# NVlabs/FoundationPose

Hardware: AMD Instinct MI355X
Metric: pose-hypotheses/sec (raster+refine+score), 252 hyp x 160x160 @ 640x480 RGB-D (higher is better)
Workload: dtype f16

## Files before the change

### foundationpose_amd/_lib.py

```python
import ctypes as C
import os

import torch

_HERE = os.path.dirname(os.path.abspath(__file__))
LIB_PATH = os.environ.get("FP_AMD_LIB") or os.path.join(_HERE, "csrc", "libfp_amd.so")
ABI_VERSION = 223
_lib = None

vp, ci, cf, cd, sz = C.c_void_p, C.c_int, C.c_float, C.c_double, C.c_size_t

SIGNATURES = {
    "fp_last_error": (C.c_char_p, []),
    "fp_version": (ci, []),
    "fp_mesh_create": (ci, [vp, vp, vp, vp, vp, vp, vp, ci, ci, ci, ci, C.POINTER(vp)]),
    "fp_mesh_destroy": (None, [vp]),
    "fp_mesh_set_create": (ci, [vp, ci, C.POINTER(vp)]),
    "fp_mesh_set_destroy": (None, [vp]),
    "fp_mesh_set_workspace_bytes": (sz, [vp, ci, ci, ci]),
    "fp_depth_erode": (ci, [vp, vp, ci, ci, ci, cf, cf, cf, vp]),
    "fp_depth_bilateral": (ci, [vp, vp, ci, ci, ci, cf, cf, cf, vp]),
    "fp_depth_to_xyz": (ci, [vp, vp, cf, ci, vp, ci, ci, vp]),
    "fp_crop_windows": (ci, [vp, vp, cd, cd, ci, ci, ci, vp, vp, vp]),
    "fp_crop_windows_multi": (ci, [vp, vp, vp, vp, ci, cd, ci, ci, ci, vp, vp, vp]),
    "fp_depth_erode_frames": (ci, [vp, vp, ci, ci, ci, ci, cf, cf, cf, vp]),
    "fp_depth_bilateral_frames": (ci, [vp, vp, ci, ci, ci, ci, cf, cf, cf, vp]),
    "fp_depth_to_xyz_frames": (ci, [vp, vp, cf, ci, vp, ci, ci, ci, vp]),
    "fp_mask_depth_stats": (ci, [vp, vp, vp, ci, ci, ci, ci, cf, vp, vp]),
    "fp_crop_windows_views": (ci, [vp, vp, vp, ci, vp, vp, ci, cd, ci, ci, ci, vp, vp, vp]),
    "fp_render_crops_views": (ci, [vp, vp, vp, vp, vp, ci, vp, vp, ci, ci, ci, ci, ci, cf, cf, cf, ci, vp, vp, vp, vp, vp, vp, vp, vp, sz, vp]),
    "fp_warp_crops_views": (ci, [vp, vp, vp, vp, vp, vp, ci, vp, vp, vp, ci, ci, ci, ci, ci, ci, ci, ci, vp, vp]),
    "fp_pose_update_views": (ci, [vp, vp, vp, ci, ci, vp, cf, vp, vp, ci, ci, vp, vp, vp, ci, vp, vp, ci, vp, cf, vp]),
    "fp_depth_agreement": (ci, [vp, vp, vp, vp, ci, ci, ci, ci, ci, ci, cf, vp, vp]),
    "fp_pose_errors_workspace_bytes": (sz, [ci, ci, ci]),
    "fp_pose_errors": (ci, [vp, ci, vp, ci, vp, vp, vp, ci, ci, ci, vp, vp, sz, vp]),
    "fp_vsd_counts": (ci, [vp, vp, vp, ci, ci, ci, ci, vp, vp, ci, ci, ci, ci, cf, vp, ci, vp, vp]),
    "fp_mspd": (ci, [vp, ci, vp, ci, vp, vp, vp, ci, ci, vp, vp, vp]),
    "fp_tsdf_integrate": (ci, [vp, vp, vp, vp, vp, ci, ci, ci, ci, ci, ci, vp, cf, cf, cf, vp, vp, vp, vp, vp]),
    "fp_tsdf_count_triangles": (ci, [vp, vp, ci, ci, ci, cf, vp, vp]),
    "fp_tsdf_emit_triangles": (ci, [vp, vp, vp, vp, ci, ci, ci, vp, cf, cf, vp, C.c_longlong, vp, vp, vp, vp, vp]),
    "fp_texture_bake": (ci, [vp, ci, vp, ci, vp, vp, vp, vp, vp, vp, ci, ci, ci, ci, ci, cf, cf, cf, vp, vp, vp]),
    "fp_workspace_bytes": (sz, [ci, ci, ci, ci, ci]),
    "fp_render_crops": (ci, [vp, vp, vp, vp, ci, ci, ci, ci, ci, cf, cf, cf, cf, ci, vp, vp, vp, vp, vp, vp, vp, vp, sz, vp]),
    "fp_render_crops_multi": (ci, [vp, vp, vp, vp, vp, vp, ci, ci, ci, ci, ci, cf, cf, cf, ci, vp, vp, vp, vp, vp, vp, vp, vp, sz, vp]),
    "fp_warp_crops": (ci, [vp, vp, vp, vp, vp, vp, cf, ci, ci, ci, ci, ci, ci, ci, vp, vp]),
    "fp_warp_crops_multi": (ci, [vp, vp, vp, vp, vp, vp, vp, vp, ci, ci, ci, ci, ci, ci, ci, ci, vp, vp]),
    "fp_pose_update": (ci, [vp, vp, vp, ci, ci, vp, cf, cf, ci, vp, vp, vp, ci, vp, vp, cf, vp]),
    "fp_pose_update_multi": (ci, [vp, vp, vp, ci, ci, vp, cf, vp, vp, ci, ci, vp, vp, vp, ci, vp, vp, cf, vp]),
    "fp_conv7x7s2_bn_relu_fwd": (ci, [vp, vp, vp, vp, vp, vp, ci, ci, ci, ci, vp]),
    "fp_igemm_f16_fwd": (ci, [vp, vp, vp, vp, vp, ci, ci, ci, ci, vp, vp]),
    "fp_pack_conv3x3_tiles_f16": (ci, [vp, vp, ci, ci, vp]),
    "fp_igemm_splitk_workspace_bytes": (sz, [ci, ci, ci]),
    "fp_igemm_f16_splitk_fwd": (ci, [vp, vp, vp, vp, vp, ci, ci, ci, ci, vp, ci, vp, sz, vp]),
    "fp_add_pe_f16_fwd": (ci, [vp, vp, vp, ci, ci, ci, vp]),
    "fp_replicate_rows_f16": (ci, [vp, vp, ci, ci, ci, ci, ci, C.c_longlong, vp]),
    "fp_replicate_segments_f16": (ci, [vp, vp, ci, ci, ci, ci, ci, C.c_longlong, vp]),
    "fp_layernorm_res_fwd": (ci, [vp, vp, vp, ci, vp, vp, vp, cf, vp, vp, ci, ci, vp]),
    "fp_pack_linear512_f16": (ci, [vp, vp, vp]),
    "fp_linear512_f16_fwd": (ci, [vp, vp, vp, vp, ci, ci, ci, vp]),
    "fp_linear_layernorm_fwd": (ci, [vp, vp, vp, vp, vp, vp, ci, vp, vp, cf, vp, vp, ci, ci, ci, ci, vp]),
    "fp_ffn_layernorm_mean_fwd": (ci, [vp, vp, vp, vp, vp, vp, vp, vp, cf, vp, vp, C.c_size_t, ci, ci, vp]),
    "fp_encoder_tail_workspace_bytes": (sz, [ci, ci]),
    "fp_encoder_tail_mean_fwd": (ci, [vp, ci, vp, vp, vp, vp, vp, vp, vp, vp, vp, vp, vp, vp, cf, vp, vp, sz, ci, ci, vp]),
    "fp_colmean_f16_fwd": (ci, [vp, vp, vp, vp, cf, vp, ci, ci, ci, vp]),
    "fp_rows_linear_fwd": (ci, [vp, vp, vp, vp, ci, ci, ci, ci, vp]),
    "fp_attention_f16_fwd": (ci, [vp, vp, ci, ci, ci, ci, ci, vp]),
    "fp_attention_segments_f16_fwd": (ci, [vp, vp, vp, ci, ci, ci, ci, ci, vp]),
    "fp_cluster_poses": (ci, [cf, cf, vp, ci, vp, ci, vp]),
}


class FpAmdError(RuntimeError):
    pass

# ... 26 lines not shown
```

### foundationpose_amd/csrc/conv_sw.hip

```cpp
#include <hip/hip_fp16.h>
#include <stdlib.h>
#include <string.h>
#include <type_traits>
#include "igemm_common.h"
#include "igemm_epilogue.h"

#ifdef FP_PROFILE_BUILD
__device__ unsigned long long sw_dbg[8];
extern "C" int fp_dbg_conv_sw(unsigned long long* out, int reset) {
  if (reset) { unsigned long long z[8] = {0, 0, 0, 0, 0, 0, ~0ull, 0}; return (int)hipMemcpyToSymbol(HIP_SYMBOL(sw_dbg), z, sizeof(z)); }
  return (int)hipMemcpyFromSymbol(out, HIP_SYMBOL(sw_dbg), 8 * sizeof(unsigned long long));
}
extern "C" int fp_dbg_conv_sw_epilogue(unsigned long long* out, int reset) {
  if (reset) { unsigned long long z[8] = {0, 0, 0, 0, 0, 0, 0, 0}; return (int)hipMemcpyToSymbol(HIP_SYMBOL(ig_epi_dbg), z, sizeof(z)); }
  return (int)hipMemcpyFromSymbol(out, HIP_SYMBOL(ig_epi_dbg), 8 * sizeof(unsigned long long));
}
#define SW_CLK(t) const unsigned long long t = wall_clock64()
#else
#define SW_CLK(t)
#endif

#ifndef SW_DEFAULT_VARIANT
#define SW_DEFAULT_VARIANT 0
#endif

namespace {

constexpr int SW_BK = 32, SW_NSTW = 4;
constexpr int sw_prows(int BM) { return BM == 256 ? 512 : 768; }

template <int N>
__device__ __forceinline__ void sw_wait_vm() {
  static_assert(N >= 0 && N < 64, "vmcnt is a 6-bit field");
  asm volatile("s_waitcnt vmcnt(%0)" ::"n"(N) : "memory");
}

__device__ __forceinline__ int sw_q(const IgemmGeom& g, int m) {
  const int b = ig_fastdiv(m, g.mulP, g.shrP);
  const int r = m - b * g.HoWo;
  const int oy = ig_fastdiv(r, g.mulW, g.shrW);
  const int ox = r - oy * g.Wo;
  return (b * g.Hp + oy) * g.Wp + ox;
}

template <int BM, int BN, int TM, bool S16>
__global__ __launch_bounds__(512, 1) void k_conv_sw(IgemmParams p) {
  constexpr int BK = SW_BK, NW = 8, THREADS = 512;
  constexpr int NWN = BN / 64;
  static_assert((BM / (32 * TM)) * NWN == NW, "8 waves");
  constexpr int ROWB = BK * 2;
  constexpr int W_BYTES = BN * ROWB;
  constexpr int SW_PROWS = sw_prows(BM);
  constexpr int SW_PATCH_BYTES = SW_PROWS * ROWB;
  constexpr int WI = BN / 16 / NW;
  constexpr int PI = SW_PROWS / 16 / NW;
  static_assert(WI >= 1 && PI >= 1 && PI <= 7 && SW_PROWS == PI * 16 * NW, "tile shape");
  constexpr int STAGES_BYTES = 2 * SW_PATCH_BYTES + SW_NSTW * W_BYTES;
  constexpr int LDS_MAIN = ig_lds_main<BM, BN>(STAGES_BYTES);
  auto swz = [](int row) { return (row >> 2) & 3; };
  auto swzp = [](int row) { return S16 ? (row >> 1) & 2 : (row >> 2) & 3; };
  extern __shared__ __attribute__((aligned(16))) unsigned char smem[];
  SW_CLK(t_start);
  unsigned char* const patch = smem;
  unsigned char* const wring = smem + 2 * SW_PATCH_BYTES;
  const int tid = threadIdx.x, lane = tid & 63;
  const int wid = __builtin_amdgcn_readfirstlane(tid >> 6);
  const int grp = wid >> 2;
  const int wm = wid / NWN, wn = wid - wm * NWN;
  float* bias_lds = reinterpret_cast<float*>(smem + LDS_MAIN);

  const int tiles_n = p.N / BN;
  const int nwg = gridDim.x;
  const int xcd = blockIdx.x & 7, loc = blockIdx.x >> 3;
  const int qd8 = nwg >> 3, r8 = nwg & 7;
  const int tile = (xcd < r8 ? xcd * (qd8 + 1) : r8 * (qd8 + 1) + (xcd - r8) * qd8) + loc;
  const int bm = tile / tiles_n, bn = tile - bm * tiles_n;
  const int m0 = bm * BM, n0 = bn * BN;
  const int Cin = p.Cin, Ktot = 9 * Cin, Wp = p.in.Wp;
  const int ncc = Cin / BK;
  ig_bias_to_lds(p, n0, bias_lds, wid, lane);

// ... 66 lines not shown
      w_off[t >> 1][t & 1] = rw * ROWB + ((fhalf ^ swz(rw)) << 4);
    }
  } else {
#pragma unroll
    for (int t = 0; t < 2; ++t) {
      const int rw = wn * 64 + t * 32 + frow;
#pragma unroll
      for (int kk = 0; kk < 2; ++kk) w_off[t][kk] = rw * ROWB + (((2 * kk + fhalf) ^ swz(rw)) << 4);
    }
  }

#pragma unroll
  for (int j = 0; j < PI; ++j) stage_patch(0, j);
  stage_w(0, 0, 0);
  stage_w(0, 1, 1);
  stage_w(0, 2, 2);
  sw_wait_vm<2 * WI>();
  __builtin_amdgcn_s_barrier();
  SW_CLK(t_cold);
  if (grp) __builtin_amdgcn_s_barrier();

  half8 fa[2][TM], fw[2][2];
  static_assert(TM == 4, "the fragment addresses of the next tap are computed behind the MFMA groups of a k-step, one per group of four");
  int anext[NFA];
#pragma unroll
  for (int t = 0; t < NFA; ++t)
    anext[t] = S16 ? arow[t] ^ ((arow[t] >> 3) & 32) : (arow[t] << 6) + ((fhalf ^ swz(arow[t])) << 4);
  auto kstep = [&](int cc, auto tap_c, auto last_c) {
    constexpr int T = decltype(tap_c)::value;
    constexpr bool LAST = decltype(last_c)::value;
    constexpr int ky = T / 3, kx = T - 3 * ky;
    const int s = cc * 9 + T;
    const unsigned char* pb = patch + (cc & 1) * SW_PATCH_BYTES;
    const unsigned char* wb = wring + (s & (SW_NSTW - 1)) * W_BYTES;
    const int shift = ky * Wp + kx;
    if constexpr (S16) {
#pragma unroll
      for (int t = 0; t < NFA; ++t) fa[t >> 2][t & 3] = *reinterpret_cast<const half8*>(pb + anext[t]);
#pragma unroll
      for (int t = 0; t < 4; ++t) fw[t >> 1][t & 1] = *reinterpret_cast<const half8*>(wb + w_off[t >> 1][t & 1]);
    } else {
#pragma unroll
      for (int t = 0; t < TM; ++t) {
        const int a0 = anext[t];
        fa[0][t] = *reinterpret_cast<const half8*>(pb + a0);
        fa[1][t] = *reinterpret_cast<const half8*>(pb + (a0 ^ 32));
      }
#pragma unroll
      for (int kk = 0; kk < 2; ++kk)
#pragma unroll
        for (int t = 0; t < 2; ++t) fw[kk][t] = *reinterpret_cast<const half8*>(wb + w_off[t][kk]);
    }
    (void)shift;
    if constexpr (!LAST) {
      if constexpr (T < PI) stage_patch(cc + 1, T);
      if constexpr (T + 3 < 9) stage_w(cc, T + 3, (s + 3) & (SW_NSTW - 1));
      else stage_w(cc + 1, T - 6, (s + 3) & (SW_NSTW - 1));
      constexpr int NP = (T < PI ? 1 : 0) + ((T >= 1 && T - 1 < PI) ? 1 : 0);
      sw_wait_vm<2 * WI + NP>();
    } else {
      if constexpr (T + 3 < 9) stage_w(cc, T + 3, (s + 3) & (SW_NSTW - 1));
      constexpr int NYOUNGER = T <= 5 ? 2 : (T == 6 ? 1 : 0);
      sw_wait_vm<NYOUNGER * WI>();
    }
    asm volatile("s_waitcnt lgkmcnt(0)" ::: "memory");
    __builtin_amdgcn_sched_barrier(0);
    __builtin_amdgcn_s_barrier();
    __builtin_amdgcn_sched_barrier(0);
    __builtin_amdgcn_s_setprio(1);
    {
      constexpr int TN = (T + 1) % 9, kyn = TN / 3, kxn = TN - 3 * kyn;
      const int shift_n = kyn * Wp + kxn;
      if constexpr (S16) {
        int sh = shift_n << 6;
        asm volatile("" : "+s"(sh));
#pragma unroll
        for (int i = 0; i < 4; ++i)
#pragma unroll
          for (int jh = 0; jh < 2; ++jh) {
#pragma unroll
            for (int j = 0; j < 4; ++j)
              acc[i][jh * 4 + j] = __builtin_amdgcn_mfma_f32_16x16x32_f16(fw[i >> 1][i & 1], fa[jh][j], acc[i][jh * 4 + j], 0, 0, 0);
            const int t = i * 2 + jh;
            const int x = arow[t] + sh;
            anext[t] = x ^ ((x >> 3) & 32);
          }
      } else {
#pragma unroll
      for (int kk = 0; kk < 2; ++kk)
#pragma unroll
        for (int i = 0; i < 2; ++i) {
#pragma unroll
          for (int j = 0; j < TM; ++j)
            acc[i][j] = __builtin_amdgcn_mfma_f32_32x32x16_f16(fw[kk][i], fa[kk][j], acc[i][j], 0, 0, 0);
          const int t = kk * 2 + i;
          {
            int ar = arow[t];
            asm volatile("" : "+v"(ar));
            const int pr = ar + shift_n;
            anext[t] = (pr << 6) + ((fhalf ^ swz(pr)) << 4);
          }
        }
      }
    }
    __builtin_amdgcn_s_setprio(0);
    __builtin_amdgcn_sched_barrier(0);
    __builtin_amdgcn_s_barrier();
    __builtin_amdgcn_sched_barrier(0);
  };
  auto chunk = [&](int cc, auto last_c) {
    kstep(cc, std::integral_constant<int, 0>{}, last_c);
    kstep(cc, std::integral_constant<int, 1>{}, last_c);
    kstep(cc, std::integral_constant<int, 2>{}, last_c);
    kstep(cc, std::integral_constant<int, 3>{}, last_c);
    kstep(cc, std::integral_constant<int, 4>{}, last_c);
    kstep(cc, std::integral_constant<int, 5>{}, last_c);
    kstep(cc, std::integral_constant<int, 6>{}, last_c);
    kstep(cc, std::integral_constant<int, 7>{}, last_c);
    kstep(cc, std::integral_constant<int, 8>{}, last_c);
  };
  for (int cc = 0; cc + 1 < ncc; ++cc) chunk(cc, std::false_type{});
  chunk(ncc - 1, std::true_type{});
  if (!grp) __builtin_amdgcn_s_barrier();
  __syncthreads();
  SW_CLK(t_loop);
  ig_epilogue<BM, BN, TM, THREADS, 0>(p, acc, smem, m0, n0, wm, wn, tid, lane, bias_lds);
#ifdef FP_PROFILE_BUILD
  asm volatile("s_waitcnt vmcnt(0)" ::: "memory");
  SW_CLK(t_end);
  if (tid == 0) {
    atomicAdd(&sw_dbg[0], t_cold - t_start); atomicAdd(&sw_dbg[1], t_loop - t_cold); atomicAdd(&sw_dbg[2], t_end - t_loop);
    atomicAdd(&sw_dbg[3], 1ull); atomicMin(&sw_dbg[6], t_start); atomicMax(&sw_dbg[7], t_end);
  }
#endif
}

constexpr int LS_PROWS = 448, LS_NSTW = 3;

template <int BM, int BN, int TM>
__global__ __launch_bounds__(256, 2) void k_conv_sw_ls(IgemmParams p) {
  constexpr int BK = SW_BK, NW = 4, THREADS = 256;
  constexpr int NWN = BN / 64;
  static_assert((BM / (32 * TM)) * NWN == NW, "4 waves");
  constexpr int ROWB = BK * 2;
  constexpr int W_BYTES = BN * ROWB;
  constexpr int PATCH_BYTES = LS_PROWS * ROWB;
  constexpr int WI = BN / 16 / NW;
  constexpr int PI = LS_PROWS / 16 / NW;
  static_assert(WI >= 1 && PI >= 1 && PI <= 8 && LS_PROWS == PI * 16 * NW, "tile shape");
// ... 142 lines not shown
  };
  chunk(0, std::false_type{}, std::true_type{});
  for (int cc = 1; cc + 1 < ncc; ++cc) chunk(cc, std::false_type{}, std::false_type{});
  chunk(ncc - 1, std::true_type{}, std::false_type{});
  __syncthreads();
  float* bias_lds = reinterpret_cast<float*>(smem + BM * BN * 2 + BM * 16);
  ig_bias_to_lds(p, n0, bias_lds, wid, lane);
  asm volatile("s_waitcnt vmcnt(0)" ::: "memory");
  ig_epilogue<BM, BN, TM, THREADS, 0>(p, acc, smem, m0, n0, wm, wn, tid, lane, bias_lds);
}

template <int BM, int BN, int TM>
int sw_ls_launch(const IgemmParams& p, hipStream_t stream) {
  constexpr int LDS = 2 * LS_PROWS * SW_BK * 2 + LS_NSTW * BN * SW_BK * 2;
  static_assert(2 * LDS <= 160 * 1024, "two workgroups per CU");
  const long long tiles = (long long)fp_cdiv(p.M, BM) * (p.N / BN);
  FP_REQUIRE(tiles < (1ll << 31), "fp_igemm_f16_fwd: too many tiles");
  FP_SET_MAX_LDS((k_conv_sw_ls<BM, BN, TM>), LDS);
  hipLaunchKernelGGL((k_conv_sw_ls<BM, BN, TM>), dim3((unsigned)tiles), dim3(256), LDS, stream, p);
  FP_CHECK_LAUNCH("fp_igemm_f16_fwd(conv_sw_ls)");
  return FP_OK;
}

template <int BM, int BN, int TM, bool S16>
int sw_launch(const IgemmParams& p, hipStream_t stream) {
  constexpr int LDS = ig_lds_main<BM, BN>(2 * sw_prows(BM) * SW_BK * 2 + SW_NSTW * BN * SW_BK * 2) + IG_BIAS_LDS;
  static_assert(LDS <= 160 * 1024, "does not fit the 160 KiB LDS");
  const long long tiles = (long long)fp_cdiv(p.M, BM) * (p.N / BN);
  FP_REQUIRE(tiles < (1ll << 31), "fp_igemm_f16_fwd: too many tiles");
  FP_SET_MAX_LDS((k_conv_sw<BM, BN, TM, S16>), LDS);
  hipLaunchKernelGGL((k_conv_sw<BM, BN, TM, S16>), dim3((unsigned)tiles), dim3(512), LDS, stream, p);
  FP_CHECK_LAUNCH("fp_igemm_f16_fwd(conv_sw)");
  return FP_OK;
}

}

static int sw_span(const IgemmGeom& g, int BM) {
  const int row_cross = (BM - 1) / g.Wo + 1, img_cross = (BM - 1) / g.HoWo + 1;
  return (BM - 1) + 2 * row_cross + (2 * g.Wp + 2) * img_cross + 2 * g.Wp + 3;
}

static int sw_variant(const IgemmParams& p) {
  int v = SW_DEFAULT_VARIANT;
#ifdef FP_PROFILE_BUILD
  static int forced = -2;
  if (forced == -2) {
    const char* e = getenv("FP_CONV_SW");
    forced = e ? (!strcmp(e, "ls") ? 1 : (!strcmp(e, "pp") ? 0 : -1)) : -1;
// ... 1 lines not shown
  if (forced >= 0) v = forced;
#endif
  if (v == 2) v = p.Cin <= 128 ? 1 : 0;
  if (v == 3) v = p.Cin <= 256 ? 1 : 0;
  if (v == 1 && sw_span(p.in, 256) > LS_PROWS) v = 0;
  return v;
}

#ifndef SW_FORCE_512
#define SW_FORCE_512 1
#endif
static bool sw_use_256(const IgemmParams& p) { return (p.N % 256) == 0 && (!SW_FORCE_512 || p.M < 2 * 512); }
static int sw_tile_rows(const IgemmParams& p) { return sw_variant(p) == 1 ? 256 : (sw_use_256(p) ? 256 : 512); }

bool fp_conv3x3_sw_applicable(const IgemmParams& p) {
  const IgemmGeom& g = p.in;
  if (p.taps != 9 || g.stride != 1 || g.off != 0 || g.bsplit != 0) return false;
  if (g.HoWo % g.Wo != 0 || g.Wp != g.Wo + 2 || g.Hp != g.HoWo / g.Wo + 2) return false;
  const int BM = sw_tile_rows(p);
  if (p.M % g.HoWo != 0 || p.M < 2 * BM) return false;
  if (p.Cin % 64 != 0 || p.N % 128 != 0) return false;
  const long long bytes = (long long)(p.M / g.HoWo) * g.Hp * g.Wp * g.cstride * 2;
  if (bytes >= (1ll << 31)) return false;
  return sw_span(g, BM) <= (sw_variant(p) == 1 ? LS_PROWS : sw_prows(BM));
}

int fp_conv3x3_sw_tile_rows(const IgemmParams& p) { return sw_tile_rows(p); }

int fp_conv3x3_sw_launch(const IgemmParams& p, hipStream_t stream) {
  if (sw_variant(p) == 1) return sw_ls_launch<256, 128, 4>(p, stream);
  if (sw_use_256(p)) return p.mfma16 ? sw_launch<256, 256, 4, true>(p, stream) : sw_launch<256, 256, 4, false>(p, stream);
  return p.mfma16 ? sw_launch<512, 128, 4, true>(p, stream) : sw_launch<512, 128, 4, false>(p, stream);
}

__global__ __launch_bounds__(256) void k_pack_conv3x3_tiles(const _Float16* __restrict__ w, _Float16* __restrict__ out, int N, int Cin) {
  const int nk = 9 * (Cin / 32);
  const long long total = (long long)N * nk * 4;
  const long long q = (long long)blockIdx.x * 256 + threadIdx.x;
  if (q >= total) return;
  const int pc = (int)(q & 3);
  const int r = (int)((q >> 2) & 127);
  const long long blk = q >> 9;
  const int s = (int)(blk % nk), bn = (int)(blk / nk);
  const int cc = s / 9, tap = s - 9 * cc;
  const int lc = pc ^ ((r >> 2) & 3);
  const half8 v = *reinterpret_cast<const half8*>(w + (size_t)(bn * 128 + r) * (9 * Cin) + tap * Cin + cc * 32 + lc * 8);
  *reinterpret_cast<half8*>(out + q * 8) = v;
}

extern "C" int fp_pack_conv3x3_tiles_f16(const void* w, void* w_tiles, int N, int Cin, void* stream) {
// ... 10 lines not shown
```

### foundationpose_amd/csrc/igemm_epilogue.h

```cpp
#pragma once
#include <type_traits>
#include "igemm_common.h"

#ifdef FP_PROFILE_BUILD
static __device__ unsigned long long ig_epi_dbg[8];
#define IG_CLK(t) const unsigned long long t = wall_clock64()
#else
#define IG_CLK(t)
#endif

#define IG_VEC_FLOATS 256
#define IG_BIAS_LDS (3 * IG_VEC_FLOATS * 4)

template <int BM, int BN>
constexpr int ig_lds_main(int stage_bytes) {
  return stage_bytes > BM * BN * 2 + BM * 16 ? stage_bytes : BM * BN * 2 + BM * 16;
}

typedef float ig_float4 __attribute__((ext_vector_type(4)));
template <int BM, int BN, int TM, int THREADS, int DBG, bool FULL, typename Acc>
__device__ __forceinline__ void ig_epilogue_body(const IgemmParams& p, Acc& acc, unsigned char* smem, int m0, int n0,
                                                 int wm, int wn, int tid, int lane, const float* bias_lds) {
  constexpr bool S16 = std::is_same<Acc, ig_float4[4][2 * TM]>::value;
  static_assert(S16 || std::is_same<Acc, float16_[2][TM]>::value, "accumulator layout");
  constexpr int CPR = BN / 8;
  constexpr int NIT = (BM * CPR) / THREADS;
  unsigned char* E = smem;
  typedef float float4_ __attribute__((ext_vector_type(4)));
  const bool round_acc = p.round_acc != 0, has_bn = p.bn_scale != nullptr;
  long long* rowY = reinterpret_cast<long long*>(smem + BM * 2 * BN);
  long long* rowR = rowY + BM;
  IG_CLK(te0);
  for (int r = tid; r < BM; r += THREADS) {
    const int m = m0 + r;
    const bool in = m < p.M;
    rowY[r] = in ? ig_row_off(p.out, m) + n0 : -1;
    if (p.R) rowR[r] = in ? ig_row_off(p.res, m) + n0 : 0;
  }
  __syncthreads();
  IG_CLK(te1);
  half8 rv[NIT];
  if (p.R) {
#pragma unroll
    for (int it = 0; it < NIT; ++it) {
      const int qd = tid + it * THREADS;
      const int ml = qd / CPR, ch = qd % CPR;
      if (FULL || rowY[ml] >= 0) rv[it] = *reinterpret_cast<const half8*>(p.R + rowR[ml] + ch * 8);
    }
  }
  IG_CLK(te2);
  auto put4 = [&](int nl, int ml, float a0, float a1, float a2, float a3, const float4_& bv, const float4_& sc, const float4_& sh) {
    half4 v;
    if (round_acc) {
      typedef _Float16 half2_ __attribute__((ext_vector_type(2)));
      const half2_ b01 = {(_Float16)bv[0], (_Float16)bv[1]}, b23 = {(_Float16)bv[2], (_Float16)bv[3]};
      half2_ t01 = {(_Float16)a0, (_Float16)a1};
      half2_ t23 = {(_Float16)a2, (_Float16)a3};
      t01 = t01 + b01;
      t23 = t23 + b23;
      if (has_bn) {
        v[0] = (_Float16)fmaf((float)t01[0], sc[0], sh[0]);
        v[1] = (_Float16)fmaf((float)t01[1], sc[1], sh[1]);
        v[2] = (_Float16)fmaf((float)t23[0], sc[2], sh[2]);
        v[3] = (_Float16)fmaf((float)t23[1], sc[3], sh[3]);
      } else {
        v[0] = t01[0]; v[1] = t01[1]; v[2] = t23[0]; v[3] = t23[1];
      }
    } else {
      v[0] = (_Float16)(a0 + bv[0]); v[1] = (_Float16)(a1 + bv[1]); v[2] = (_Float16)(a2 + bv[2]); v[3] = (_Float16)(a3 + bv[3]);
    }
// ... 24 lines not shown
  } else {
#pragma unroll
    for (int i = 0; i < 2; ++i) {
#pragma unroll
      for (int g = 0; g < 4; ++g) {
        const int nl = wn * 64 + i * 32 + 8 * g + 4 * (lane >> 5);
        float4_ bv, sc, sh;
        vecs(nl, bv, sc, sh);
#pragma unroll
        for (int j = 0; j < TM; ++j) {
          const int ml = wm * (32 * TM) + j * 32 + (lane & 31);
          put4(nl, ml, acc[i][j][g * 4 + 0], acc[i][j][g * 4 + 1], acc[i][j][g * 4 + 2], acc[i][j][g * 4 + 3], bv, sc, sh);
        }
      }
    }
  }
  __syncthreads();
  IG_CLK(te3);
  const half8 zero = {0, 0, 0, 0, 0, 0, 0, 0};
#pragma unroll
  for (int it = 0; it < NIT; ++it) {
    const int qd = tid + it * THREADS;
    const int ml = qd / CPR, ch = qd % CPR;
    const long long yo = rowY[ml];
    if (!FULL && yo < 0) continue;
    half8 v = *reinterpret_cast<const half8*>(E + ml * (2 * BN) + ((ch ^ (ml & 15)) << 4));
    if (p.R) v = v + rv[it];
    if (p.relu) v = __builtin_elementwise_max(v, zero);
    *reinterpret_cast<half8*>(p.Y + yo + ch * 8) = v;
    if (p.Ype) {
      const int m = m0 + ml;
      const float* per = p.pe + (size_t)(m % p.pe_period) * p.N + n0 + ch * 8;
      const float4_ e0 = *reinterpret_cast<const float4_*>(per), e1 = *reinterpret_cast<const float4_*>(per + 4);
      half8 w;
#pragma unroll
      for (int e = 0; e < 4; ++e) { w[e] = (_Float16)((float)v[e] + e0[e]); w[4 + e] = (_Float16)((float)v[4 + e] + e1[e]); }
      *reinterpret_cast<half8*>(p.Ype + (size_t)m * p.N + n0 + ch * 8) = w;
    }
  }
#ifdef FP_PROFILE_BUILD
  IG_CLK(te4);
  if (tid == 0) {
    atomicAdd(&ig_epi_dbg[0], te1 - te0); atomicAdd(&ig_epi_dbg[1], te2 - te1); atomicAdd(&ig_epi_dbg[2], te3 - te2);
    atomicAdd(&ig_epi_dbg[3], te4 - te3); atomicAdd(&ig_epi_dbg[4], 1ull);
  }
#endif
}

template <int BM, int BN, int TM, int THREADS, int DBG = 0, typename Acc>
__device__ __forceinline__ void ig_epilogue(const IgemmParams& p, Acc& acc, unsigned char* smem, int m0, int n0,
                                            int wm, int wn, int tid, int lane, const float* bias_lds) {
  if (m0 + BM <= p.M) ig_epilogue_body<BM, BN, TM, THREADS, DBG, true>(p, acc, smem, m0, n0, wm, wn, tid, lane, bias_lds);
  else ig_epilogue_body<BM, BN, TM, THREADS, DBG, false>(p, acc, smem, m0, n0, wm, wn, tid, lane, bias_lds);
}
__device__ __forceinline__ void ig_bias_to_lds(const IgemmParams& p, int n0, float* bias_lds, int wid, int lane) {
  if (wid > 2) return;
  const float* src = wid == 0 ? p.bias : (wid == 1 ? p.bn_scale : p.bn_shift);
  float* dst = bias_lds + wid * IG_VEC_FLOATS;
  if (src) {
    const __amdgpu_buffer_rsrc_t rs = __builtin_amdgcn_make_buffer_rsrc(const_cast<float*>(src), 0, p.N * 4, 0x00020000);
    __builtin_amdgcn_raw_ptr_buffer_load_lds(rs, (__attribute__((address_space(3))) void*)dst, 16, lane * 16, n0 * 4, 0, 0);
  } else if (wid == 0) {
    typedef float f4 __attribute__((ext_vector_type(4)));
    *reinterpret_cast<f4*>(dst + lane * 4) = f4{0.f, 0.f, 0.f, 0.f};
  }
}
```

### foundationpose_amd/csrc/raster.hip

```cpp
#include <hip/hip_fp16.h>
#include "fp_common.h"

#define FP_SUBPIX 16.0f
#define FP_GUARD_LO (-8192.0f)
#define FP_GUARD_HI (24575.0f)
#define FP_ZNEAR 0.001f
#define FP_ZMAXF 4095.0f
#define FP_ZSCALEF 1048576.0f
#define FP_VTX_INVALID 0x80008000u
#define FP_KEY_EMPTY 0xFFFFFFFFFFFFFFFFull
#define FP_RASTER_THREADS 256

struct HypConst {
  float P[12];
  float umin, vmin, ax, ay;
  float fx, sk, cx, fy, cy;
};

struct RenderOut {
  void* A;
  float* color;
  float* depth;
  float* xyz;
  float* normal;
// ... 501 lines not shown
static inline size_t ws_align(size_t x) { return (x + 255) & ~(size_t)255; }

struct WsLayout { size_t vr, va, counts, lists, total; int nstrips; bool ids16; };

static WsLayout ws_layout(int N, int V, int T, int oh) {
  WsLayout L;
  L.nstrips = fp_cdiv(oh, FP_STRIP_ROWS);
  L.ids16 = T <= 65535;
  size_t o = 0;
  L.vr = o; o = ws_align(o + (size_t)N * V * sizeof(VtxRec));
  L.va = o; o = ws_align(o + (size_t)N * V * sizeof(VtxAttr));
  L.counts = o; o = ws_align(o + (size_t)N * L.nstrips * sizeof(int));
  L.lists = o; o = ws_align(o + (size_t)N * L.nstrips * T * (L.ids16 ? 2 : 4));
  L.total = o;
  return L;
}

extern "C" size_t fp_workspace_bytes(int N, int V, int T, int oh, int ow) {
  (void)ow;
  if (N <= 0 || V <= 0 || T <= 0 || oh <= 0) return 0;
  return ws_layout(N, V, T, oh).total;
}

extern "C" size_t fp_mesh_set_workspace_bytes(const fp_mesh_set* set, int N, int oh, int ow) {
  if (!set) return 0;
  return fp_workspace_bytes(N, set->maxV, set->maxT, oh, ow);
}

template <bool MULTI, bool VIEWS = false>
static int render_launch(const char* name, const fp_mesh& one, const MeshTable& tab, int maxV, int maxT, const float* poses,
                         const float* bbox2d, const float* K9, int H, int W, int N, int oh, int ow, float w_ambient,
                         float w_diffuse, float inv_r, float xyz_thr, int flags, const RenderOut& out, void* workspace,
                         size_t workspace_bytes, hipStream_t st, const fp_views& vt = fp_views{nullptr, nullptr, 0}) {
  FP_REQUIRE(oh > 0 && ow > 0 && oh <= 1024 && ow <= 1024, "%s: output size %dx%d unsupported (max 1024)", name, oh, ow);
  FP_REQUIRE(bbox2d || (oh == H && ow == W), "%s: full-frame render needs oh==H and ow==W", name);
  FP_REQUIRE(N <= 65535, "%s: N=%d exceeds the grid limit; chunk the batch", name, N);
  const WsLayout L = ws_layout(N, maxV, maxT, oh);
  if (!workspace || workspace_bytes < L.total) {
    fp_set_error("%s: workspace too small (%zu < %zu bytes, see fp_workspace_bytes)", name, workspace_bytes, L.total);
    return FP_ERR_WORKSPACE;
  }
  fp_k9 K = {};
  if (!VIEWS)
    for (int i = 0; i < 9; ++i) K.v[i] = K9[i];
  unsigned char* w8 = (unsigned char*)workspace;
  RenderWs ws;
  ws.vr = (VtxRec*)(w8 + L.vr); ws.va = (VtxAttr*)(w8 + L.va); ws.counts = (int*)(w8 + L.counts);
  ws.lists16 = L.ids16 ? (unsigned short*)(w8 + L.lists) : nullptr;
  ws.lists32 = L.ids16 ? nullptr : (int*)(w8 + L.lists);
  ws.vstride = maxV; ws.tstride = maxT;
  const dim3 gv(fp_cdiv(maxV, 256), N), gb(fp_cdiv(maxT, 256), N), gr(L.nstrips, N);
  const size_t lds = (size_t)FP_STRIP_ROWS * ow * sizeof(unsigned long long) + 16 + FP_BIG_MAX * sizeof(BigTri);
  if constexpr (VIEWS) {
    hipLaunchKernelGGL((k_vertex<MULTI, fp_views>), gv, dim3(256), 0, st, one, tab, poses, bbox2d, K, H, W, oh, ow, L.nstrips, ws, vt);
    FP_CHECK_LAUNCH("fp_render_crops_views(vertex)");
    hipLaunchKernelGGL((k_bin<MULTI, fp_views>), gb, dim3(256), 0, st, one, tab, oh, ow, L.nstrips, ws, vt);
    FP_CHECK_LAUNCH("fp_render_crops_views(bin)");
    FP_SET_MAX_LDS((k_raster<MULTI, fp_views>), 160 * 1024);
    hipLaunchKernelGGL((k_raster<MULTI, fp_views>), gr, dim3(FP_RASTER_THREADS), lds, st, one, tab, poses, bbox2d, K, H, W, oh, ow,
                       L.nstrips, w_ambient, w_diffuse, inv_r, xyz_thr, flags, out, ws, vt);
  } else {
    hipLaunchKernelGGL(k_vertex<MULTI>, gv, dim3(256), 0, st, one, tab, poses, bbox2d, K, H, W, oh, ow, L.nstrips, ws);
    FP_CHECK_LAUNCH(MULTI ? "fp_render_crops_multi(vertex)" : "fp_render_crops(vertex)");
    hipLaunchKernelGGL(k_bin<MULTI>, gb, dim3(256), 0, st, one, tab, oh, ow, L.nstrips, ws);
    FP_CHECK_LAUNCH(MULTI ? "fp_render_crops_multi(bin)" : "fp_render_crops(bin)");
    FP_SET_MAX_LDS(k_raster<MULTI>, 160 * 1024);
    hipLaunchKernelGGL(k_raster<MULTI>, gr, dim3(FP_RASTER_THREADS), lds, st, one, tab, poses, bbox2d, K, H, W, oh, ow, L.nstrips,
                       w_ambient, w_diffuse, inv_r, xyz_thr, flags, out, ws);
  }
  FP_CHECK_LAUNCH(name);
  return FP_OK;
}

extern "C" int fp_render_crops(const fp_mesh* mesh, const float* poses, const float* bbox2d, const float* K9, int H,
                               int W, int N, int oh, int ow, float w_ambient, float w_diffuse, float mesh_diameter,
// ... 56 lines not shown
```

### include/fp_amd.h

```cpp
#ifndef FP_AMD_H
#define FP_AMD_H

#include <stddef.h>
#include <stdint.h>

#ifdef __cplusplus
extern "C" {
#endif

typedef enum {
  FP_OK = 0,
  FP_ERR_INVALID_ARG = -1,
  FP_ERR_WORKSPACE = -2,
  FP_ERR_LAUNCH = -3,
  FP_ERR_UNSUPPORTED = -4
} fp_status;

#define FP_FLAG_NORMALIZE_XYZ 1
#define FP_FLAG_OUT_F16 2

#define FP_MODE_REFINE 0
#define FP_MODE_SCORE 1

#define FP_ROT_AXIS_ANGLE 0
#define FP_ROT_6D 1
#define FP_TRANS_TRACKNET 0
#define FP_TRANS_DEEPIM 1
#define FP_TRANS_RAW 2

#define FP_SUBPIXEL_BITS 4
#define FP_ZBUF_STEPS_PER_METRE 1048576
#define FP_ZBUF_EMPTY 0xFFFFFFFFu

typedef struct fp_mesh fp_mesh;
typedef struct fp_mesh_set fp_mesh_set;

const char* fp_last_error(void);
#define FP_AMD_ABI_VERSION 223
int fp_version(void);

int fp_mesh_create(const float* pos , const float* nrm , const int32_t* faces ,
                   const float* uv , const int32_t* uv_idx ,
                   const float* tex , const float* vcol , int V, int T, int Ht,
                   int Wt, fp_mesh** out);
void fp_mesh_destroy(fp_mesh* mesh);

#define FP_MESH_SET_MAX_ELEMS (1 << 26)
int fp_mesh_set_create(const fp_mesh* const* meshes , int M, fp_mesh_set** out);
void fp_mesh_set_destroy(fp_mesh_set* set);
size_t fp_mesh_set_workspace_bytes(const fp_mesh_set* set, int N, int oh, int ow);

int fp_depth_erode(const float* depth , float* out , int H, int W, int radius,
                   float depth_diff_thres, float ratio_thres, float zfar, void* stream);
int fp_depth_bilateral(const float* depth , float* out , int H, int W, int radius,
                       float zfar, float sigmaD, float sigmaR, void* stream);
int fp_depth_to_xyz(const float* depth , const double* K , float zfar,
                    int f64_internal, float* xyz , int H, int W, void* stream);

int fp_depth_erode_frames(const float* depth , float* out , int H, int W, int V, int radius,
                          float depth_diff_thres, float ratio_thres, float zfar, void* stream);
int fp_depth_bilateral_frames(const float* depth , float* out , int H, int W, int V, int radius,
// ... 48 lines not shown
                           float* pos , float* col , float* nrm , void* stream);
#define FP_TEXTURE_BAKE_MAX_TEXELS 16
#define FP_TEXTURE_BAKE_MAX_SIDE 16384
int fp_texture_bake(const float* pos , int Nv, const int32_t* faces , int F,
                    const float* vertex_color , const float* depth ,
                    const float* rgb , const uint8_t* masks ,
                    const float* ob_in_cams , const double* Ks , int V, int H, int W, int T, int Bx, float tol,
                    float min_cos, float min_depth, float* tex , uint8_t* coverage , void* stream);
int fp_pose_update_views(const float* trans , const float* rot , const float* poses_in ,
                         int rot_rep, int normalize_xyz, const float* trans_normalizer , float rot_normalizer,
                         const double* diameters , const int32_t* obj , int M, int N,
                         float* poses_out , float* trans_delta_out , float* rot_delta_out ,
                         int trans_rep, const float* Ks , const int32_t* view , int V,
                         const float* tf_to_crops , float input_w, void* stream);

int fp_crop_windows(const float* poses , const double* K , double mesh_diameter,
                    double crop_ratio, int out_w, int out_h, int N, float* tf_to_crops ,
                    float* bbox2d , void* stream);
int fp_crop_windows_multi(const float* poses , const double* K , const double* diameters ,
                          const int32_t* obj , int M, double crop_ratio, int out_w, int out_h, int N,
                          float* tf_to_crops , float* bbox2d , void* stream);

size_t fp_workspace_bytes(int N, int V, int T, int oh, int ow);

int fp_render_crops(const fp_mesh* mesh, const float* poses , const float* bbox2d ,
                    const float* K9 , int H, int W, int N, int oh, int ow, float w_ambient,
                    float w_diffuse, float mesh_diameter, float xyz_thr, int flags, void* A ,
                    float* color , float* depth , float* xyz , float* normal ,
                    uint32_t* zbuf , int32_t* tri_id , void* workspace ,
                    size_t workspace_bytes, void* stream);

int fp_render_crops_multi(const fp_mesh_set* set, const int32_t* obj , const double* diameters ,
                          const float* poses , const float* bbox2d , const float* K9 ,
                          int H, int W, int N, int oh, int ow, float w_ambient, float w_diffuse, float xyz_thr, int flags,
                          void* A , float* color , float* depth , float* xyz , float* normal ,
                          uint32_t* zbuf , int32_t* tri_id , void* workspace , size_t workspace_bytes,
                          void* stream);

int fp_warp_crops(const float* rgb , const float* xyz_map , const float* depth ,
                  const float* tf_to_crops , const float* K9 ,
                  const float* poses , float mesh_diameter, int flags, int mode, int H, int W,
                  int N, int oh, int ow, void* B , void* stream);

int fp_warp_crops_multi(const float* rgb , const float* xyz_map , const float* depth ,
                        const float* tf_to_crops , const float* K9 , const float* poses ,
                        const double* diameters , const int32_t* obj , int M, int flags, int mode, int H,
// ... 26 lines not shown
#define FP_IGEMM_ROUND_ACC 2

#define FP_IGEMM_MFMA_16X16X32 16
#define FP_IGEMM_MFMA_32X32X16 32

typedef struct {
  const float* bias;
  const float* bn_scale;
  const float* bn_shift;
  const void* residual;
  const fp_igemm_geom* r_geom;
  int flags;
  const float* pe;
  int pe_period;
  void* y_pe;
  const void* w_tiles;
} fp_igemm_epilogue;

int fp_igemm_f16_fwd(const void* x , const fp_igemm_geom* x_geom , const void* w , void* y ,
                     const fp_igemm_geom* y_geom , int M, int N, int Cin, int taps,
                     const fp_igemm_epilogue* epilogue , void* stream);

int fp_pack_conv3x3_tiles_f16(const void* w , void* w_tiles , int N, int Cin, void* stream);

size_t fp_igemm_splitk_workspace_bytes(int M, int N, int splits);
int fp_igemm_f16_splitk_fwd(const void* x , const fp_igemm_geom* x_geom , const void* w , void* y ,
                            const fp_igemm_geom* y_geom , int M, int N, int Cin, int taps,
                            const fp_igemm_epilogue* epilogue , int splits, void* workspace ,
                            size_t workspace_bytes, void* stream);

int fp_add_pe_f16_fwd(const void* tok , const float* pe , void* out , int M, int S, int D, void* stream);

int fp_replicate_rows_f16(const void* src , void* dst , int copies, int rows, int channels, int src_row_stride,
                          int dst_row_stride, long long dst_copy_stride, void* stream);

int fp_replicate_segments_f16(void* buf , const int32_t* seg_offsets , int segments, int images, int pixels,
                              int channels, int pixel_stride, long long image_stride, void* stream);

int fp_layernorm_res_fwd(const float* x32 , const void* tok16 , const float* pe , int S,
                         const void* branch16 , const float* gamma , const float* beta , float eps,
                         float* y32 , void* y16 , int M, int D, void* stream);

int fp_pack_linear512_f16(const void* w16 , void* packed , void* stream);

int fp_linear512_f16_fwd(const void* x16 , const void* w_packed , const float* bias , void* y16 ,
                         int M, int N, int relu, void* stream);
// ... 48 lines not shown
```

Baseline: 7535.

## Slim conv3x3 sliding-window epilogue LDS and hand-schedule MFMA address math

The conv3x3 sliding-window kernel's epilogue now stores output row offsets as 32-bit deltas from a tile base, and reuses the staging area for residual row offsets. This shrinks the LDS footprint, and a guard rejects outputs whose offsets would overflow 32 bits. The S16 inner loop replaces compiler-scheduled MFMA builtins with inline-asm MFMAs interleaved with the next tap's address arithmetic, splitting the swizzle XOR into a separately kept flip term. New entry points expose the raster and conv LDS sizes, and the ABI version is bumped. The aim is lower LDS use, possibly better occupancy, and address math hidden behind MFMA latency, at the cost of an extra barrier in the epilogue and fragile volatile asm scheduling.

```diff
diff --git a/foundationpose_amd/_lib.py b/foundationpose_amd/_lib.py
--- a/foundationpose_amd/_lib.py
+++ b/foundationpose_amd/_lib.py
@@ -5,7 +5,7 @@
 
 _HERE = os.path.dirname(os.path.abspath(__file__))
 LIB_PATH = os.environ.get("FP_AMD_LIB") or os.path.join(_HERE, "csrc", "libfp_amd.so")
-ABI_VERSION = 223
+ABI_VERSION = 224
 _lib = None
 
 vp, ci, cf, cd, sz = C.c_void_p, C.c_int, C.c_float, C.c_double, C.c_size_t
@@ -41,6 +41,7 @@
     "fp_tsdf_emit_triangles": (ci, [vp, vp, vp, vp, ci, ci, ci, vp, cf, cf, vp, C.c_longlong, vp, vp, vp, vp, vp]),
     "fp_texture_bake": (ci, [vp, ci, vp, ci, vp, vp, vp, vp, vp, vp, ci, ci, ci, ci, ci, cf, cf, cf, vp, vp, vp]),
     "fp_workspace_bytes": (sz, [ci, ci, ci, ci, ci]),
+    "fp_raster_lds_bytes": (sz, [ci]),
     "fp_render_crops": (ci, [vp, vp, vp, vp, ci, ci, ci, ci, ci, cf, cf, cf, cf, ci, vp, vp, vp, vp, vp, vp, vp, vp, sz, vp]),
     "fp_render_crops_multi": (ci, [vp, vp, vp, vp, vp, vp, ci, ci, ci, ci, ci, cf, cf, cf, ci, vp, vp, vp, vp, vp, vp, vp, vp, sz, vp]),
     "fp_warp_crops": (ci, [vp, vp, vp, vp, vp, vp, cf, ci, ci, ci, ci, ci, ci, ci, vp, vp]),
@@ -50,6 +51,7 @@
     "fp_conv7x7s2_bn_relu_fwd": (ci, [vp, vp, vp, vp, vp, vp, ci, ci, ci, ci, vp]),
     "fp_igemm_f16_fwd": (ci, [vp, vp, vp, vp, vp, ci, ci, ci, ci, vp, vp]),
     "fp_pack_conv3x3_tiles_f16": (ci, [vp, vp, ci, ci, vp]),
+    "fp_conv3x3_sw_lds_bytes": (ci, []),
     "fp_igemm_splitk_workspace_bytes": (sz, [ci, ci, ci]),
     "fp_igemm_f16_splitk_fwd": (ci, [vp, vp, vp, vp, vp, ci, ci, ci, ci, vp, ci, vp, sz, vp]),
     "fp_add_pe_f16_fwd": (ci, [vp, vp, vp, ci, ci, ci, vp]),
diff --git a/foundationpose_amd/csrc/conv_sw.hip b/foundationpose_amd/csrc/conv_sw.hip
--- a/foundationpose_amd/csrc/conv_sw.hip
+++ b/foundationpose_amd/csrc/conv_sw.hip
@@ -33,6 +33,11 @@
 __device__ __forceinline__ void sw_wait_vm() {
   static_assert(N >= 0 && N < 64, "vmcnt is a 6-bit field");
   asm volatile("s_waitcnt vmcnt(%0)" ::"n"(N) : "memory");
+}
+
+typedef float sw_float4 __attribute__((ext_vector_type(4)));
+__device__ __forceinline__ void sw_mfma16(sw_float4& acc, const half8& a, const half8& b) {
+  asm volatile("v_mfma_f32_16x16x32_f16 %0, %1, %2, %0" : "+v"(acc) : "v"(a), "v"(b));
 }
 
 __device__ __forceinline__ int sw_q(const IgemmGeom& g, int m) {
@@ -56,7 +61,7 @@
   constexpr int PI = SW_PROWS / 16 / NW;
   static_assert(WI >= 1 && PI >= 1 && PI <= 7 && SW_PROWS == PI * 16 * NW, "tile shape");
   constexpr int STAGES_BYTES = 2 * SW_PATCH_BYTES + SW_NSTW * W_BYTES;
-  constexpr int LDS_MAIN = ig_lds_main<BM, BN>(STAGES_BYTES);
+  constexpr int LDS_MAIN = ig_lds_main_slim<BM, BN>(STAGES_BYTES);
   auto swz = [](int row) { return (row >> 2) & 3; };
   auto swzp = [](int row) { return S16 ? (row >> 1) & 2 : (row >> 2) & 3; };
   extern __shared__ __attribute__((aligned(16))) unsigned char smem[];
@@ -169,10 +174,12 @@
 
   half8 fa[2][TM], fw[2][2];
   static_assert(TM == 4, "the fragment addresses of the next tap are computed behind the MFMA groups of a k-step, one per group of four");
-  int anext[NFA];
-#pragma unroll
-  for (int t = 0; t < NFA; ++t)
-    anext[t] = S16 ? arow[t] ^ ((arow[t] >> 3) & 32) : (arow[t] << 6) + ((fhalf ^ swz(arow[t])) << 4);
+  int anext[NFA], aflip[NFA];
+#pragma unroll
+  for (int t = 0; t < NFA; ++t) {
+    anext[t] = S16 ? arow[t] : (arow[t] << 6) + ((fhalf ^ swz(arow[t])) << 4);
+    aflip[t] = S16 ? (arow[t] >> 3) & 32 : 0;
+  }
   auto kstep = [&](int cc, auto tap_c, auto last_c) {
     constexpr int T = decltype(tap_c)::value;
     constexpr bool LAST = decltype(last_c)::value;
@@ -183,7 +190,7 @@
     const int shift = ky * Wp + kx;
     if constexpr (S16) {
 #pragma unroll
-      for (int t = 0; t < NFA; ++t) fa[t >> 2][t & 3] = *reinterpret_cast<const half8*>(pb + anext[t]);
+      for (int t = 0; t < NFA; ++t) fa[t >> 2][t & 3] = *reinterpret_cast<const half8*>(pb + (anext[t] ^ aflip[t]));
 #pragma unroll
       for (int t = 0; t < 4; ++t) fw[t >> 1][t & 1] = *reinterpret_cast<const half8*>(wb + w_off[t >> 1][t & 1]);
     } else {
@@ -225,12 +232,16 @@
         for (int i = 0; i < 4; ++i)
 #pragma unroll
           for (int jh = 0; jh < 2; ++jh) {
-#pragma unroll
-            for (int j = 0; j < 4; ++j)
-              acc[i][jh * 4 + j] = __builtin_amdgcn_mfma_f32_16x16x32_f16(fw[i >> 1][i & 1], fa[jh][j], acc[i][jh * 4 + j], 0, 0, 0);
             const int t = i * 2 + jh;
-            const int x = arow[t] + sh;
-            anext[t] = x ^ ((x >> 3) & 32);
+            int x, y;
+            sw_mfma16(acc[i][jh * 4 + 0], fw[i >> 1][i & 1], fa[jh][0]);
+            asm volatile("v_add_u32 %0, %1, %2" : "=v"(x) : "s"(sh), "v"(arow[t]));
+            sw_mfma16(acc[i][jh * 4 + 1], fw[i >> 1][i & 1], fa[jh][1]);
+            asm volatile("v_lshrrev_b32 %0, 3, %1" : "=v"(y) : "v"(x));
+            sw_mfma16(acc[i][jh * 4 + 2], fw[i >> 1][i & 1], fa[jh][2]);
+            asm volatile("v_and_b32 %0, 32, %0" : "+v"(y));
+            sw_mfma16(acc[i][jh * 4 + 3], fw[i >> 1][i & 1], fa[jh][3]);
+            anext[t] = x; aflip[t] = y;
           }
       } else {
 #pragma unroll
@@ -271,7 +282,7 @@
   if (!grp) __builtin_amdgcn_s_barrier();
   __syncthreads();
   SW_CLK(t_loop);
-  ig_epilogue<BM, BN, TM, THREADS, 0>(p, acc, smem, m0, n0, wm, wn, tid, lane, bias_lds);
+  ig_epilogue<BM, BN, TM, THREADS, 0, true>(p, acc, smem, m0, n0, wm, wn, tid, lane, bias_lds);
 #ifdef FP_PROFILE_BUILD
   asm volatile("s_waitcnt vmcnt(0)" ::: "memory");
   SW_CLK(t_end);
@@ -460,9 +471,15 @@
   return FP_OK;
 }
 
+constexpr int sw_lds_bytes(int BM, int BN) {
+  return (BM == 256 ? ig_lds_main_slim<256, 256>(2 * sw_prows(256) * SW_BK * 2 + SW_NSTW * 256 * SW_BK * 2)
+                    : ig_lds_main_slim<512, 128>(2 * sw_prows(512) * SW_BK * 2 + SW_NSTW * 128 * SW_BK * 2)) + IG_BIAS_LDS;
+}
+
 template <int BM, int BN, int TM, bool S16>
 int sw_launch(const IgemmParams& p, hipStream_t stream) {
-  constexpr int LDS = ig_lds_main<BM, BN>(2 * sw_prows(BM) * SW_BK * 2 + SW_NSTW * BN * SW_BK * 2) + IG_BIAS_LDS;
+  static_assert((BM == 256 && BN == 256) || (BM == 512 && BN == 128), "tile shapes of sw_lds_bytes");
+  constexpr int LDS = sw_lds_bytes(BM, BN);
   static_assert(LDS <= 160 * 1024, "does not fit the 160 KiB LDS");
   const long long tiles = (long long)fp_cdiv(p.M, BM) * (p.N / BN);
   FP_REQUIRE(tiles < (1ll << 31), "fp_igemm_f16_fwd: too many tiles");
@@ -510,10 +527,15 @@
   if (p.Cin % 64 != 0 || p.N % 128 != 0) return false;
   const long long bytes = (long long)(p.M / g.HoWo) * g.Hp * g.Wp * g.cstride * 2;
   if (bytes >= (1ll << 31)) return false;
+  const IgemmGeom& o = p.out;
+  const long long imgs = o.bsplit > 0 ? o.bsplit : p.M / g.HoWo, groups = o.bsplit > 0 ? (p.M / g.HoWo) / o.bsplit + 1 : 0;
+  if (imgs * o.Hp * o.Wp * o.cstride + o.coff + groups * (long long)o.cgroup >= (1ll << 31)) return false;
   return sw_span(g, BM) <= (sw_variant(p) == 1 ? LS_PROWS : sw_prows(BM));
 }
 
 int fp_conv3x3_sw_tile_rows(const IgemmParams& p) { return sw_tile_rows(p); }
+
+extern "C" int fp_conv3x3_sw_lds_bytes(void) { return sw_lds_bytes(512, 128); }
 
 int fp_conv3x3_sw_launch(const IgemmParams& p, hipStream_t stream) {
   if (sw_variant(p) == 1) return sw_ls_launch<256, 128, 4>(p, stream);
diff --git a/foundationpose_amd/csrc/igemm_epilogue.h b/foundationpose_amd/csrc/igemm_epilogue.h
--- a/foundationpose_amd/csrc/igemm_epilogue.h
+++ b/foundationpose_amd/csrc/igemm_epilogue.h
@@ -17,8 +17,14 @@
   return stage_bytes > BM * BN * 2 + BM * 16 ? stage_bytes : BM * BN * 2 + BM * 16;
 }
 
+template <int BM, int BN>
+constexpr int ig_lds_main_slim(int stage_bytes) {
+  return stage_bytes > BM * BN * 2 + BM * 4 ? stage_bytes : BM * BN * 2 + BM * 4;
+}
+#define IG_ROW_NONE ((int)0x80000000)
+
 typedef float ig_float4 __attribute__((ext_vector_type(4)));
-template <int BM, int BN, int TM, int THREADS, int DBG, bool FULL, typename Acc>
+template <int BM, int BN, int TM, int THREADS, int DBG, bool FULL, bool SLIM, typename Acc>
 __device__ __forceinline__ void ig_epilogue_body(const IgemmParams& p, Acc& acc, unsigned char* smem, int m0, int n0,
                                                  int wm, int wn, int tid, int lane, const float* bias_lds) {
   constexpr bool S16 = std::is_same<Acc, ig_float4[4][2 * TM]>::value;
@@ -29,12 +35,16 @@
   typedef float float4_ __attribute__((ext_vector_type(4)));
   const bool round_acc = p.round_acc != 0, has_bn = p.bn_scale != nullptr;
   long long* rowY = reinterpret_cast<long long*>(smem + BM * 2 * BN);
-  long long* rowR = rowY + BM;
+  long long* rowR = SLIM ? reinterpret_cast<long long*>(smem) : rowY + BM;
+  int* rowY32 = reinterpret_cast<int*>(smem + BM * 2 * BN);
+  const long long baseY = SLIM ? ig_row_off(p.out, m0) + n0 : 0;
+  auto row_exists = [&](int ml) { return SLIM ? rowY32[ml] != IG_ROW_NONE : rowY[ml] >= 0; };
   IG_CLK(te0);
   for (int r = tid; r < BM; r += THREADS) {
     const int m = m0 + r;
     const bool in = m < p.M;
-    rowY[r] = in ? ig_row_off(p.out, m) + n0 : -1;
+    if constexpr (SLIM) rowY32[r] = in ? (int)(ig_row_off(p.out, m) + n0 - baseY) : IG_ROW_NONE;
+    else rowY[r] = in ? ig_row_off(p.out, m) + n0 : -1;
     if (p.R) rowR[r] = in ? ig_row_off(p.res, m) + n0 : 0;
   }
   __syncthreads();
@@ -45,7 +55,13 @@
     for (int it = 0; it < NIT; ++it) {
       const int qd = tid + it * THREADS;
       const int ml = qd / CPR, ch = qd % CPR;
-      if (FULL || rowY[ml] >= 0) rv[it] = *reinterpret_cast<const half8*>(p.R + rowR[ml] + ch * 8);
+      if (FULL || row_exists(ml)) rv[it] = *reinterpret_cast<const half8*>(p.R + rowR[ml] + ch * 8);
+    }
+    if constexpr (SLIM) {
+      __builtin_amdgcn_sched_barrier(0);
+      asm volatile("s_waitcnt lgkmcnt(0)" ::: "memory");
+      __builtin_amdgcn_s_barrier();
+      __builtin_amdgcn_sched_barrier(0);
     }
   }
   IG_CLK(te2);
@@ -116,8 +132,8 @@
   for (int it = 0; it < NIT; ++it) {
     const int qd = tid + it * THREADS;
     const int ml = qd / CPR, ch = qd % CPR;
-    const long long yo = rowY[ml];
-    if (!FULL && yo < 0) continue;
+    if (!FULL && !row_exists(ml)) continue;
+    const long long yo = SLIM ? baseY + rowY32[ml] : rowY[ml];
     half8 v = *reinterpret_cast<const half8*>(E + ml * (2 * BN) + ((ch ^ (ml & 15)) << 4));
     if (p.R) v = v + rv[it];
     if (p.relu) v = __builtin_elementwise_max(v, zero);
@@ -141,11 +157,11 @@
 #endif
 }
 
-template <int BM, int BN, int TM, int THREADS, int DBG = 0, typename Acc>
+template <int BM, int BN, int TM, int THREADS, int DBG = 0, bool SLIM = false, typename Acc>
 __device__ __forceinline__ void ig_epilogue(const IgemmParams& p, Acc& acc, unsigned char* smem, int m0, int n0,
                                             int wm, int wn, int tid, int lane, const float* bias_lds) {
-  if (m0 + BM <= p.M) ig_epilogue_body<BM, BN, TM, THREADS, DBG, true>(p, acc, smem, m0, n0, wm, wn, tid, lane, bias_lds);
-  else ig_epilogue_body<BM, BN, TM, THREADS, DBG, false>(p, acc, smem, m0, n0, wm, wn, tid, lane, bias_lds);
+  if (m0 + BM <= p.M) ig_epilogue_body<BM, BN, TM, THREADS, DBG, true, SLIM>(p, acc, smem, m0, n0, wm, wn, tid, lane, bias_lds);
+  else ig_epilogue_body<BM, BN, TM, THREADS, DBG, false, SLIM>(p, acc, smem, m0, n0, wm, wn, tid, lane, bias_lds);
 }
 __device__ __forceinline__ void ig_bias_to_lds(const IgemmParams& p, int n0, float* bias_lds, int wid, int lane) {
   if (wid > 2) return;
diff --git a/foundationpose_amd/csrc/raster.hip b/foundationpose_amd/csrc/raster.hip
--- a/foundationpose_amd/csrc/raster.hip
+++ b/foundationpose_amd/csrc/raster.hip
@@ -547,6 +547,11 @@
   return ws_layout(N, V, T, oh).total;
 }
 
+extern "C" size_t fp_raster_lds_bytes(int ow) {
+  if (ow <= 0) return 0;
+  return (size_t)FP_STRIP_ROWS * ow * sizeof(unsigned long long) + 16 + FP_BIG_MAX * sizeof(BigTri);
+}
+
 extern "C" size_t fp_mesh_set_workspace_bytes(const fp_mesh_set* set, int N, int oh, int ow) {
   if (!set) return 0;
   return fp_workspace_bytes(N, set->maxV, set->maxT, oh, ow);
@@ -575,7 +580,7 @@
   ws.lists32 = L.ids16 ? nullptr : (int*)(w8 + L.lists);
   ws.vstride = maxV; ws.tstride = maxT;
   const dim3 gv(fp_cdiv(maxV, 256), N), gb(fp_cdiv(maxT, 256), N), gr(L.nstrips, N);
-  const size_t lds = (size_t)FP_STRIP_ROWS * ow * sizeof(unsigned long long) + 16 + FP_BIG_MAX * sizeof(BigTri);
+  const size_t lds = fp_raster_lds_bytes(ow);
   if constexpr (VIEWS) {
     hipLaunchKernelGGL((k_vertex<MULTI, fp_views>), gv, dim3(256), 0, st, one, tab, poses, bbox2d, K, H, W, oh, ow, L.nstrips, ws, vt);
     FP_CHECK_LAUNCH("fp_render_crops_views(vertex)");
diff --git a/include/fp_amd.h b/include/fp_amd.h
--- a/include/fp_amd.h
+++ b/include/fp_amd.h
@@ -36,7 +36,7 @@
 typedef struct fp_mesh_set fp_mesh_set;
 
 const char* fp_last_error(void);
-#define FP_AMD_ABI_VERSION 223
+#define FP_AMD_ABI_VERSION 224
 int fp_version(void);
 
 int fp_mesh_create(const float* pos , const float* nrm , const int32_t* faces ,
@@ -131,6 +131,7 @@
                           float* tf_to_crops , float* bbox2d , void* stream);
 
 size_t fp_workspace_bytes(int N, int V, int T, int oh, int ow);
+size_t fp_raster_lds_bytes(int ow);
 
 int fp_render_crops(const fp_mesh* mesh, const float* poses , const float* bbox2d ,
                     const float* K9 , int H, int W, int N, int oh, int ow, float w_ambient,
@@ -203,6 +204,7 @@
                      const fp_igemm_epilogue* epilogue , void* stream);
 
 int fp_pack_conv3x3_tiles_f16(const void* w , void* w_tiles , int N, int Cin, void* stream);
+int fp_conv3x3_sw_lds_bytes(void);
 
 size_t fp_igemm_splitk_workspace_bytes(int M, int N, int splits);
 int fp_igemm_f16_splitk_fwd(const void* x , const fp_igemm_geom* x_geom , const void* w , void* y ,
```

Measured after the change: 7651 (median of 6 runs). 1.5% higher.
